# vrettasm/VGPA

Hardware: AMD Instinct MI355X
Metric: fwd+bwd sweeps/sec (free-energy+grad eval), Lorenz96 D=40 N=1000 (higher is better)
Workload: dtype f64; 1 GPU; Lorenz96 D=40, RK4, Np=1001 (BASELINE configs[2]); batch_per_gpu=512, kernels=mfma

## Files before the change

### vgpa_amd/csrc/energy.hip

```cpp
#include "vgpa_internal.h"
#include "energy_small.h"
#include "chol_wave.h"

namespace vgpa {
namespace {

constexpr int NT = 256;

__global__ void __launch_bounds__(NT) k_energy_1d(EnergyArgs a) {
  const int t = blockIdx.x * NT + threadIdx.x;
  const int prob = blockIdx.y;
  if (t >= a.Np) return;
  const size_t o = (size_t)prob * a.Np + t;
  const double la = a.A[(size_t)prob * a.strideA + t], ob = a.b[(size_t)prob * a.strideB + t], m = a.m[o], s = a.S[o];
  Energy1d r;
  const double th = a.theta_v ? a.theta_v[(size_t)prob * kMaxTheta] : a.theta[0];
  const double sg = a.sigma1_v ? a.sigma1_v[prob] : a.sigma1;
  if (a.model == VGPA_MODEL_OU) energy_1d<VGPA_MODEL_OU>(th, sg, la, ob, m, s, r);
  else energy_1d<VGPA_MODEL_DW>(th, sg, la, ob, m, s, r);
  if (a.hyp_only) { a.hyp[o] = r.hyp; return; }
  a.e_t[o] = r.e_t;
  a.Ef[o] = r.ef;
  if (a.Edf) a.Edf[o] = r.edf;
  a.dEm[o] = r.dm;
  a.dEs[o] = r.ds;
  if (a.hyp) a.hyp[o] = r.hyp;
}

__global__ void __launch_bounds__(64) k_energy_l63(EnergyArgs a) {
  const int t = blockIdx.x * 64 + threadIdx.x;
  const int prob = blockIdx.y;
  if (t >= a.Np) return;
  const size_t o = (size_t)prob * a.Np + t;
  const double* At = a.A + (size_t)prob * a.strideA + (size_t)t * 9;
  const double* bt = a.b + (size_t)prob * a.strideB + (size_t)t * 3;
  const double* mt = a.m + o * 3;
  const double* St = a.S + o * 9;
  double Av[9], bv[3], mv[3], Sv[9], isg[3];
  const double* th = a.theta_v ? a.theta_v + (size_t)prob * kMaxTheta : a.theta;
  const double* isgp = a.isg + (size_t)prob * a.isg_stride;
#pragma unroll
  for (int e = 0; e < 9; e++) { Av[e] = At[e]; Sv[e] = St[e]; }
#pragma unroll
  for (int i = 0; i < 3; i++) { bv[i] = bt[i]; mv[i] = mt[i]; isg[i] = isgp[i]; }
  EnergyL63 r;
  if (a.hyp) energy_l63<true>(th, isg, Av, bv, mv, Sv, r); else energy_l63<false>(th, isg, Av, bv, mv, Sv, r);
  if (a.hyp_only) {
    double* hp = a.hyp + o * 6;
#pragma unroll
    for (int i = 0; i < 6; i++) hp[i] = r.hyp[i];
    return;
  }
  a.e_t[o] = r.e_t;
  double* dm = a.dEm + o * 3;
  dm[0] = r.dm[0]; dm[1] = r.dm[1]; dm[2] = r.dm[2];
  double* ds = a.dEs + o * 9;
  ds[0] = r.ds[0]; ds[1] = r.ds[1]; ds[2] = r.ds[2];
  ds[3] = r.ds[1]; ds[4] = r.ds[3]; ds[5] = r.ds[4];
  ds[6] = r.ds[2]; ds[7] = r.ds[4]; ds[8] = r.ds[5];
  double* ef = a.Ef + o * 3;
  ef[0] = r.ef[0]; ef[1] = r.ef[1]; ef[2] = r.ef[2];
  if (a.hyp) {
    double* hp = a.hyp + o * 6;
#pragma unroll
    for (int i = 0; i < 6; i++) hp[i] = r.hyp[i];
  }
  if (a.Edf) {
    double* e = a.Edf + o * 9;
    const double vS = th[0], vR = th[1], vB = th[2];
    e[0] = -vS; e[1] = vS; e[2] = 0.0;
    e[3] = vR - mv[2]; e[4] = -1.0; e[5] = -mv[0];
    e[6] = mv[1]; e[7] = mv[0]; e[8] = -vB;
  }
}

__device__ __forceinline__ int wrap(int i, int n) { return i < 0 ? i + n : (i >= n ? i - n : i); }

__device__ __forceinline__ void wave_sync() {
  __builtin_amdgcn_fence(__ATOMIC_RELEASE, "wavefront");
  __builtin_amdgcn_wave_barrier();
  __builtin_amdgcn_fence(__ATOMIC_ACQUIRE, "wavefront");
}

__device__ __forceinline__ double lane_value(double v, int j) {
  const int lo = __builtin_amdgcn_readlane(__double2loint(v), j);
  const int hi = __builtin_amdgcn_readlane(__double2hiint(v), j);
  return __hiloint2double(hi, lo);
}

using cholw::chol_panel_pivots;
using cholw::rsqrt_pos;

__device__ __forceinline__ double wave_sum(double v) {
#pragma unroll
  for (int o = 32; o > 0; o >>= 1) v += __shfl_xor(v, o, 64);
  return v;
}

template <int NB>
struct WaveGemmGeo {
  static constexpr int NQ = NB / 4, REM = NB % 4, G = REM ? 4 / REM : 0;
  static constexpr int NLEFT = REM ? (NB + G - 1) / G : 0;
  static constexpr int NU = NB * NQ + NLEFT;
};

template <int NB, int MODE, int TRI = 0>
__device__ __forceinline__ void wave_gemm(const double* __restrict__ Aop, const double* __restrict__ Bm, int LD,
                                          double (&acc)[WaveGemmGeo<NB>::NU], const double* __restrict__ bscale = nullptr) {
  using g = WaveGemmGeo<NB>;
  const int l = threadIdx.x & 63, r4 = l >> 4, c4 = l & 3, b = (l >> 2) & 3;
  constexpr int rem = g::REM ? g::REM : 1;
#pragma unroll
  for (int u = 0; u < g::NU; u++) acc[u] = 0.0;
  const double* pa = Aop + r4 * LD + c4;
  const double* pb = Bm + r4 * LD;
  const int colq = l & 15;
  const int coll = 4 * (4 * g::NQ + b % rem) + c4;
  const int ileft = b / rem;
#pragma unroll
  for (int kk = 0; kk < NB; kk++) {
    const double bs = bscale ? bscale[4 * kk + r4] : 1.0;
    double bq[g::NQ > 0 ? g::NQ : 1];
#pragma unroll
    for (int q = 0; q < g::NQ; q++)
      if (kk >= 4 * q) bq[q] = bscale ? bs * pb[kk * 4 * LD + 16 * q + colq] : pb[kk * 4 * LD + 16 * q + colq];
    double bl = 0.0;
    if (g::NLEFT > 0 && kk >= 4 * g::NQ) bl = bscale ? bs * pb[kk * 4 * LD + coll] : pb[kk * 4 * LD + coll];
#pragma unroll
    for (int I = 0; I < NB; I++) {
      if (MODE == 1 && kk < I) continue;
      bool any = false;
#pragma unroll
      for (int q = 0; q < g::NQ; q++) any = any || (kk >= 4 * q && !(TRI == 1 && 4 * q + 3 < I) && !(TRI == 2 && 4 * q > I));
      if (!any) continue;
      const double af = pa[kk * 4 * LD + 4 * I];
#pragma unroll
      for (int q = 0; q < g::NQ; q++)
        if (kk >= 4 * q && !(TRI == 1 && 4 * q + 3 < I) && !(TRI == 2 && 4 * q > I)) acc[q * NB + I] = __builtin_amdgcn_mfma_f64_4x4x4f64(af, bq[q], acc[q * NB + I], 0, 0, 0);
    }
    if (g::NLEFT > 0 && kk >= 4 * g::NQ) {
#pragma unroll
      for (int v = 0; v < g::NLEFT; v++) {
        if (MODE == 1 && kk < v * g::G) continue;
        if (TRI == 2 && v * g::G + g::G - 1 < 4 * g::NQ) continue;
        int ib = v * g::G + ileft;
        ib = ib < NB ? ib : NB - 1;
        const double af = pa[kk * 4 * LD + 4 * ib];
        acc[NB * g::NQ + v] = __builtin_amdgcn_mfma_f64_4x4x4f64(af, bl, acc[NB * g::NQ + v], 0, 0, 0);
      }
    }
  }
}

template <int NB>
__device__ __forceinline__ void wave_gemm_elem(int u, int& row, int& col, bool& ok) {
  using g = WaveGemmGeo<NB>;
  const int l = threadIdx.x & 63, r4 = l >> 4, c4 = l & 3, b = (l >> 2) & 3;
  constexpr int rem = g::REM ? g::REM : 1;
  int Ib, Jb;
  if (u < NB * g::NQ) {
    const int q = u / NB;
    Ib = u - q * NB; Jb = 4 * q + b; ok = true;
  } else {
    const int v = u - NB * g::NQ;
    Ib = v * g::G + b / rem; Jb = 4 * g::NQ + b % rem;
    ok = (b < g::G * g::REM) && (Ib < NB);
  }
  row = 4 * Ib + r4; col = 4 * Jb + c4;
}

struct L96Lds {
  double *Lm, *Gm, *mv, *bv, *am, *sg, *vv, *dl, *qq, *rd;
};

__host__ __device__ inline int l96_dp(int D) { return 4 * ((D + 3) / 4); }
__host__ __device__ inline int l96_ld(int D) { return l96_dp(D) + 1; }
__host__ __device__ inline size_t l96_lds_doubles(int D) {
  return (size_t)2 * l96_dp(D) * l96_ld(D) + 7 * (size_t)l96_dp(D) + (2 * D + 1) + 8 + 4 * (size_t)l96_dp(D);
}

template <int NB>
__global__ void __launch_bounds__(64) k_energy_l96(EnergyArgs a) {
  extern __shared__ __attribute__((aligned(16))) double smem[];
  const int D = a.D, M = 2 * D + 1;
  constexpr int Dp = 4 * NB, LD = Dp + 1;
  const int l = threadIdx.x;
  const long long wid = blockIdx.x;
  const int prob = (int)(wid / a.Np), t = (int)(wid - (long long)prob * a.Np);
  const size_t o = (size_t)prob * a.Np + t;
  L96Lds S;
  S.Lm = smem; S.Gm = S.Lm + Dp * LD; S.mv = S.Gm + Dp * LD; S.bv = S.mv + Dp; S.am = S.bv + Dp; S.sg = S.am + Dp;
  S.dl = S.sg + Dp; S.qq = S.dl + Dp; S.rd = S.qq + Dp; S.vv = S.rd + Dp;
  const double* At = a.A + (size_t)prob * a.strideA + (size_t)t * D * D;
  const double* St = a.S + o * D * D;
  const double theta = a.theta_v ? lds_const(a.theta_v, prob * kMaxTheta) : a.theta[0];
  const double kappa = 1.05 * D, c = D + kappa;
  const bool act = l < D;
  const bool pad = l < Dp;
  const int li = pad ? l : Dp - 1;

  for (int e = l; e < Dp * LD; e += 64) { S.Lm[e] = 0.0; S.Gm[e] = 0.0; }
  if (pad) { S.mv[l] = 0.0; S.bv[l] = 0.0; S.sg[l] = 0.0; S.am[l] = 0.0; S.dl[l] = 0.0; S.qq[l] = 0.0; S.rd[l] = 1.0; }
  wave_sync();
  {
    constexpr int EPL = (Dp * Dp + 63) / 64;
    const int DD = D * D;
    const unsigned magic = ((1u << 20) + (unsigned)D - 1u) / (unsigned)D;
#pragma unroll
    for (int q0 = 0; q0 < EPL; q0 += 9) {
      double sv[9], av[9];
#pragma unroll
      for (int u = 0; u < 9; u++) {
        const int e = l + 64 * (q0 + u);
        const bool in = (q0 + u < EPL) && (e < DD);
        sv[u] = in ? St[e] : 0.0;
        av[u] = in ? At[e] : 0.0;
      }
#pragma unroll
      for (int u = 0; u < 9; u++) {
        const int e = l + 64 * (q0 + u);
        if ((q0 + u < EPL) && (e < DD)) {
          const int r = (int)(((unsigned)e * magic) >> 20), cc = e - r * D;
          S.Lm[r * LD + cc] = c * sv[u];
          S.Gm[cc * LD + r] = av[u];
        }
      }
    }
  }
  if (l >= D && pad) S.Lm[l * LD + l] = 1.0;
  if (act) { S.mv[l] = a.m[o * D + l]; S.bv[l] = a.b[(size_t)prob * a.strideB + (size_t)t * D + l]; S.sg[l] = a.isg[(size_t)prob * a.isg_stride + l]; }
  wave_sync();

  const int r4 = l >> 4, c4 = l & 3, b = (l >> 2) & 3;
  bool bad = false;
  double myrd = 1.0;
  const double* lrow_b = S.Lm + (4 * b + c4) * LD + r4;
  double* lout_b = S.Lm + (4 * b + r4) * LD + c4;
#pragma unroll
  for (int p = 0; p < NB; p++) {
    const int j0 = 4 * p;
    if (p > 0) {
      const double* brow = S.Lm + (j0 + c4) * LD + r4;
#pragma unroll
      for (int u = 0; p + 4 * u < NB; u++) {
        const bool full = p + 4 * u + 3 < NB;
        const bool rowok = full || (p + 4 * u + b < NB);
        const double* arow = full ? lrow_b + 4 * (p + 4 * u) * LD
                                  : S.Lm + (4 * (rowok ? p + 4 * u + b : NB - 1) + c4) * LD + r4;
        double uacc = 0.0;
#pragma unroll
        for (int kk = 0; kk < p; kk++) uacc = __builtin_amdgcn_mfma_f64_4x4x4f64(arow[4 * kk], brow[4 * kk], uacc, 0, 0, 0);
        if (rowok) lout_b[4 * (p + 4 * u) * LD + j0] -= uacc;
      }
      wave_sync();
    }
    chol_panel_pivots<LD>(S.Lm, myrd, j0, l, li, pad);
    wave_sync();
  }
  if (pad) S.rd[l] = myrd;
  wave_sync();
  bad = __any(!(myrd > 0.0 && myrd < __builtin_inf()));
  if (bad) {
    if (l == 0) atomicOr(a.status + prob, 1);
    return;
  }

  double* xdiag = S.vv + (2 * D + 1) + 7;
  if (l < NB) {
    const double* tb = S.Lm + (4 * l) * LD + 4 * l;
    const double x00 = S.rd[4 * l], x11 = S.rd[4 * l + 1], x22 = S.rd[4 * l + 2], x33 = S.rd[4 * l + 3];
    const double t10 = tb[LD], t20 = tb[2 * LD], t21 = tb[2 * LD + 1], t30 = tb[3 * LD], t31 = tb[3 * LD + 1], t32 = tb[3 * LD + 2];
    const double x10 = -(t10 * x00) * x11;
    const double x21 = -(t21 * x11) * x22;
    const double x32 = -(t32 * x22) * x33;
    const double x20 = -(t20 * x00 + t21 * x10) * x22;
    const double x31 = -(t31 * x11 + t32 * x21) * x33;
    const double x30 = -(t30 * x00 + t31 * x10 + t32 * x20) * x33;
    double* xo = xdiag + 16 * l;
    xo[0] = x00; xo[1] = 0.0; xo[2] = 0.0; xo[3] = 0.0;
    xo[4] = x10; xo[5] = x11; xo[6] = 0.0; xo[7] = 0.0;
    xo[8] = x20; xo[9] = x21; xo[10] = x22; xo[11] = 0.0;
    xo[12] = x30; xo[13] = x31; xo[14] = x32; xo[15] = x33;
  }
  {
    double s = 0.0;
#pragma unroll
    for (int k = 0; k < Dp; k++) s = __builtin_fma(S.Gm[k * LD + li], S.mv[k], s);
    if (act) { S.am[l] = s; if (a.Am) a.Am[o * D + l] = s; }
    double acc[WaveGemmGeo<NB>::NU];
    wave_gemm<NB, 0>(S.Gm, S.Lm, LD, acc);
    wave_sync();
#pragma unroll
    for (int u = 0; u < WaveGemmGeo<NB>::NU; u++) {
      int row, col; bool ok;
      wave_gemm_elem<NB>(u, row, col, ok);
      if (ok) S.Gm[row * LD + col] = acc[u];
    }
  }
  wave_sync();

  double vplus = 0.0, vminus = 0.0, v0 = 0.0, r0sq = 0.0;
  const bool hyper = a.hyp != nullptr;
  {
    auto col_of = [&](int q) { return q == 0 ? 0 : (q <= D ? q - 1 : q - 1 - D); };
    auto sgn_of = [&](int q) { return q == 0 ? 0.0 : (q <= D ? 1.0 : -1.0); };
    auto chi = [&](int q, int i) { return S.mv[i] + sgn_of(q) * S.Lm[i * LD + col_of(q)]; };
    const int jc = act ? l : 0;
    const int pP = 1 + jc, pM = 1 + D + jc;
    const int pPm = pP - 1, pPp = pP + 1;
    const int pMm = pM - 1, pMp = wrap(pM + 1, M);
    double am2 = chi(pPm, D - 2), am1 = chi(pPm, D - 1), a0 = chi(pP, 0), a1 = chi(pP, 1);
    double bm2 = chi(pMm, D - 2), bm1 = chi(pMm, D - 1), b0 = chi(pM, 0), b1 = chi(pM, 1);
    const double* lcol = S.Lm + jc;
    const double* gcol = S.Gm + jc;
#pragma unroll
    for (int i = 0; i < Dp; i++) {
      if (i >= D) break;
      const double gi = gcol[i * LD], ami = S.am[i], bvi = S.bv[i], sgi = S.sg[i];
      const double ra = ((a1 - am2) * am1 - a0 + theta) + (ami + gi) - bvi;
      const double rb = ((b1 - bm2) * bm1 - b0 + theta) + (ami - gi) - bvi;
      vplus = __builtin_fma(sgi, ra * ra, vplus);
      vminus = __builtin_fma(sgi, rb * rb, vminus);
      if (hyper && act) S.Gm[i * LD + jc] = ra * ra + rb * rb;
      am2 = am1; am1 = a0; a0 = a1;
      bm2 = bm1; bm1 = b0; b0 = b1;
      const int in = i + 2;
      if (in < D) {
        const double mi = S.mv[in], li2 = lcol[in * LD];
        a1 = mi + li2; b1 = mi - li2;
      } else {
        a1 = chi(pPp, in - D); b1 = chi(pMp, in - D);
      }
    }
    if (act) {
      const int i = l;
      const double xm2 = (i >= 2) ? S.mv[i - 2] : chi(M - 1, D - 2 + i);
      const double xm1 = (i >= 1) ? S.mv[i - 1] : chi(M - 1, D - 1);
      const double x1 = (i + 1 < D) ? S.mv[i + 1] : chi(1, 0);
      const double r0 = ((x1 - xm2) * xm1 - S.mv[i] + theta) + S.am[i] - S.bv[i];
      r0sq = r0 * r0;
      v0 = S.sg[i] * r0sq;
    }
    v0 = wave_sum(v0);
  }
  const double w0 = kappa / c, w1 = 1.0 / (2.0 * c);
  if (hyper) {
    wave_sync();
    if (act) {
      double sm = 0.0;
      for (int j = 0; j < D; j++) sm += S.Gm[l * LD + j];
      const int i = l, ip1 = wrap(i + 1, D), im1 = wrap(i - 1, D), im2 = wrap(i - 2, D);
      const double efi = (St[ip1 * D + im1] - St[im2 * D + im1]) + (S.mv[ip1] - S.mv[im2]) * S.mv[im1] - S.mv[i] + theta;
      double* hp = a.hyp + o * 2 * D;
      hp[i] = efi + S.am[i] - S.bv[i];
      hp[D + i] = w0 * r0sq + w1 * sm;
    }
  }
  const double e_part = act ? (vplus + vminus) : 0.0;
  const double e_t = 0.5 * (w0 * v0 + w1 * wave_sum(e_part));
  if (act) {
    S.dl[l] = w1 * (vplus - vminus);
    S.qq[l] = 0.5 * c * (w1 * (vplus + vminus)) - e_t;
  }
  if (l == 0) a.e_t[o] = e_t;
  wave_sync();

  const double* l4_a = S.Lm + c4 * LD + r4;
  const double* xd_a = xdiag + 4 * c4 + r4;
  const double* xd_d = xdiag + 4 * r4 + c4;
#pragma unroll
  for (int I = 0; I < NB; I++) {
    const double* arow = l4_a + 4 * I * LD;
    const double xd = xd_a[16 * I];
    const double xdd = xd_d[16 * I];
#pragma unroll
    for (int u = 0; 4 * u < NB; u++) {
      const int Jb = 4 * u + b;
      const bool colok = (4 * u + 3 < NB) || (Jb < NB);
      double* xcol = S.Gm + r4 * LD + 4 * (colok ? Jb : NB - 1) + c4;
      double xo = 0.0;
      if (4 * u <= I) {
        double tacc = 0.0;
#pragma unroll
        for (int K = 4 * u; K < I; K++) tacc = __builtin_amdgcn_mfma_f64_4x4x4f64(arow[4 * K], xcol[4 * K * LD], tacc, 0, 0, 0);
        const double prod = __builtin_amdgcn_mfma_f64_4x4x4f64(xd, tacc, 0.0, 0, 0, 0);
        xo = (Jb < I) ? -prod : ((Jb == I) ? xdd : 0.0);
      }
      if (colok) xcol[4 * I * LD] = xo;
    }
    wave_sync();
  }

  {
    double s = 0.0;
    for (int k = 0; k < Dp; k++) s = __builtin_fma(S.Gm[k * LD + li], S.dl[k], s);
    if (act) a.dEm[o * D + l] = 0.5 * c * s;
  }
  double* ds = a.dEs + o * D * D;
  {
    double acc[WaveGemmGeo<NB>::NU];
    wave_gemm<NB, 1>(S.Gm, S.Gm, LD, acc, S.qq);
#pragma unroll
    for (int u = 0; u < WaveGemmGeo<NB>::NU; u++) {
      int row, col; bool ok;
      wave_gemm_elem<NB>(u, row, col, ok);
      if (ok && row < D && col < D && (row <= col || !a.ds_upper)) ds[row * D + col] = 0.5 * c * acc[u];
    }
  }

  if (act) {
    const int i = l, ip1 = wrap(i + 1, D), im1 = wrap(i - 1, D), im2 = wrap(i - 2, D);
    const double cxx = St[ip1 * D + im1] - St[im2 * D + im1];
    a.Ef[o * D + i] = cxx + (S.mv[ip1] - S.mv[im2]) * S.mv[im1] - S.mv[i] + theta;
  }
  if (a.Edf) {
    double* ed = a.Edf + o * D * D;
    for (int e = l; e < D * D; e += 64) {
      const int k = e / D, j = e - k * D;
      const int kp1 = wrap(k + 1, D), km1 = wrap(k - 1, D), km2 = wrap(k - 2, D);
      double v = 0.0;
      if (j == k) v = -1.0;
      if (j == kp1) v = S.mv[km1];
      if (j == km2) v = -S.mv[km1];
      if (j == km1) v = S.mv[kp1] - S.mv[km2];
      ed[e] = v;
    }
  }
}

__host__ __device__ inline bool l96r_compact(int D) { return (D + 3) / 4 == 10; }
__host__ __device__ inline size_t l96r_lds_doubles(int D) {
  const size_t dp = l96_dp(D);
  if (l96r_compact(D)) return dp * l96_ld(D) + 5 * dp;
  return dp * l96_ld(D) + 6 * dp + 9 * dp;
}
template <int R>
__device__ __forceinline__ double row_ror_blocks(double v) {
  typedef int i2_t __attribute__((ext_vector_type(2)));
  i2_t x = __builtin_bit_cast(i2_t, v), y;
  y[0] = __builtin_amdgcn_mov_dpp(x[0], 0x120 + 4 * R, 0xf, 0xf, false);
  y[1] = __builtin_amdgcn_mov_dpp(x[1], 0x120 + 4 * R, 0xf, 0xf, false);
  return __builtin_bit_cast(double, y);
}

struct TriRowTab { unsigned char r[2080]; };
constexpr TriRowTab make_tri_row_tab() {
  TriRowTab t{};
  int e = 0;
  for (int r = 0; r < 64; r++)
    for (int c = 0; c <= r; c++) t.r[e++] = (unsigned char)r;
  return t;
}
__device__ __constant__ TriRowTab kTriRow = make_tri_row_tab();

template <int NB, bool TG = false>
__global__ void __launch_bounds__(64) __attribute__((amdgpu_waves_per_eu(NB <= 10 ? 3 : 2, NB <= 10 ? 3 : 2))) k_energy_l96_r(EnergyArgs a) {
  extern __shared__ __attribute__((aligned(16))) double smem[];
  const int D = a.D, M = 2 * D + 1;
  constexpr int Dp = 4 * NB, LD = Dp + 1, NUU = (NB + 3) / 4;
  const int l = threadIdx.x;
  const long long wid = blockIdx.x;
  const int prob = (int)(wid / a.Np);
  const int t = (int)(wid - (long long)prob * a.Np);
  const size_t o = (size_t)prob * a.Np + t;
  L96Lds S;
  constexpr bool CMP = (NB == 10);
  S.Lm = smem; S.Gm = nullptr; S.mv = S.Lm + Dp * LD; S.bv = S.mv + Dp; S.am = S.bv + Dp; S.sg = nullptr;
  S.dl = S.am + Dp; S.qq = S.dl + Dp; S.rd = CMP ? nullptr : S.qq + Dp; S.vv = CMP ? nullptr : S.rd + Dp;
  double* pv = S.vv;
  double* pw = CMP ? nullptr : pv + 4 * Dp;
  double* gb2 = CMP ? nullptr : pw + 4 * Dp;
  double* xdiag = pv;
  auto cg2 = [&](int j) -> double* { return S.Lm + j * LD + Dp; };
  auto cps = [&](int minus, int j) -> double* { return S.Lm + (4 + 2 * minus + (j >= 20 ? 1 : 0)) * LD + (j >= 20 ? j : 20 + j); };
  auto cxd = [&](int I, int r, int c) -> double* { return S.Lm + ((I < 6 ? 0 : 4) + r) * LD + 4 * (I < 6 ? I + 4 : I - 1) + c; };
  const double* At = a.A + (size_t)prob * a.strideA + (size_t)t * D * D;
  const bool spk = a.s_packed != 0;
  const int PK = tri_off(D);
  const double* St = a.S + o * (spk ? PK : D * D);
  const double theta = a.theta_v ? lds_const(a.theta_v, prob * kMaxTheta) : a.theta[0];
  const double kappa = 1.05 * D, c = D + kappa;
  const bool act = l < D;
  const bool pad = l < Dp;
  const int li = pad ? l : Dp - 1;
  const int r4 = l >> 4, c4 = l & 3, b = (l >> 2) & 3;

  constexpr int NUE = 0;
  double af[NUU][NB];
  const int klim = (D - r4 + 3) >> 2;
  auto load_af = [&](int u) {
    const int row = 16 * u + (l & 15);
    const double* ap = At + row * D + r4;
    const int kl = row < D ? klim : 0;
#pragma unroll
    for (int K = 0; K < NB; K++) af[u][K] = (K < kl) ? ap[4 * K] : 0.0;
  };

  double sxa = 0.0, sxb = 0.0, v_m = 0.0, v_b = 0.0, v_sg = 0.0;
  double nsxa = 0.0, nsxb = 0.0;
  const int f_ip1 = wrap(l + 1, D), f_im1 = wrap(l - 1, D), f_im2 = wrap(l - 2, D);
  if (act) v_sg = a.isg[(size_t)prob * a.isg_stride + l];
  auto load_vectors = [&]() {
    if (act) {
      sxa = St[f_ip1 * D + f_im1];
      sxb = St[f_im2 * D + f_im1];
      v_m = a.m[o * D + l];
      v_b = a.b[(size_t)prob * a.strideB + (size_t)t * D + l];
    }
  };
  constexpr int EPK = (Dp * (Dp + 1) / 2 + 63) / 64;
  double sv[EPK];
  int rr[EPK];
  auto request = [&](int tn) {
    const size_t on = (size_t)prob * a.Np + tn;
    const double* Sn = a.S + on * PK;
#pragma unroll
    for (int q = 0; q < EPK; q++) {
      const int e = l + 64 * q;
      sv[q] = e < PK ? Sn[e] : 0.0;
      rr[q] = kTriRow.r[e < PK ? e : 0];
    }
    if (act) {
      nsxa = Sn[tri_idx(f_ip1, f_im1)];
      nsxb = Sn[tri_idx(f_im2, f_im1)];
      v_m = a.m[on * D + l];
      v_b = a.b[(size_t)prob * a.strideB + (size_t)tn * D + l];
    }
  };
  if (spk) request(t);

  if (spk) {
    if (D != Dp) {
      for (int e = l; e < Dp * LD; e += 64) S.Lm[e] = 0.0;
      wave_sync();
    }
    sxa = nsxa; sxb = nsxb;
#pragma unroll
    for (int q = 0; q < EPK; q++) {
      const int e = l + 64 * q;
      if (e < PK) {
        const int r = rr[q];
        S.Lm[r * LD + (e - tri_off(r))] = c * sv[q];
      }
    }
  } else if (D == Dp) {
    constexpr int RCH = Dp <= 44 ? Dp : 32;
    const double* sp = St + li;
#pragma unroll
    for (int q0 = 0; q0 < Dp; q0 += RCH) {
      double sv[RCH];
#pragma unroll
      for (int u = 0; u < RCH; u++) sv[u] = (q0 + u < Dp) ? sp[(q0 + u) * Dp] : 0.0;
      if (q0 == 0) load_vectors();
      if (pad) {
#pragma unroll
        for (int u = 0; u < RCH; u++)
          if (q0 + u < Dp) S.Lm[(q0 + u) * LD + l] = c * sv[u];
      }
    }
  } else {
    load_vectors();
    for (int e = l; e < Dp * LD; e += 64) S.Lm[e] = 0.0;
    wave_sync();
    constexpr int EPL = (Dp * Dp + 63) / 64;
    constexpr int CH = (NB <= 11) ? EPL : 13;
    const int DD = D * D;
    const unsigned magic = ((1u << 20) + (unsigned)D - 1u) / (unsigned)D;
#pragma unroll
    for (int q0 = 0; q0 < EPL; q0 += CH) {
      double sv[CH];
#pragma unroll
      for (int u = 0; u < CH; u++) {
        const int e = l + 64 * (q0 + u);
        const bool in = (q0 + u < EPL) && (e < DD);
        sv[u] = in ? St[e] : 0.0;
      }
#pragma unroll
      for (int u = 0; u < CH; u++) {
        const int e = l + 64 * (q0 + u);
        if ((q0 + u < EPL) && (e < DD)) {
          const int r = (int)(((unsigned)e * magic) >> 20), cc = e - r * D;
          S.Lm[r * LD + cc] = c * sv[u];
        }
      }
    }
  }
  if (l >= D && pad) S.Lm[l * LD + l] = 1.0;
  if (pad) { S.mv[l] = v_m; S.bv[l] = v_b; S.am[l] = 0.0; }
  wave_sync();

  bool bad = false;
  double myrd = 1.0;
  const double* lrow_b = S.Lm + (4 * b + c4) * LD + r4;
  double* lout_b = S.Lm + (4 * b + r4) * LD + c4;
#pragma unroll
  for (int p = 0; p < NB; p++) {
    const int j0 = 4 * p;
    if (p > 0) {
      const double* brow = S.Lm + (j0 + c4) * LD + r4;
#pragma unroll
      for (int u = 0; p + 4 * u < NB; u++) {
        const bool full = p + 4 * u + 3 < NB;
        const bool rowok = full || (p + 4 * u + b < NB);
        const double* arow = full ? lrow_b + 4 * (p + 4 * u) * LD
                                  : S.Lm + (4 * (rowok ? p + 4 * u + b : NB - 1) + c4) * LD + r4;
        double uacc = 0.0;
#pragma unroll
        for (int kk = 0; kk < p; kk++) uacc = __builtin_amdgcn_mfma_f64_4x4x4f64(arow[4 * kk], brow[4 * kk], uacc, 0, 0, 0);
        if (rowok) lout_b[4 * (p + 4 * u) * LD + j0] -= uacc;
      }
      wave_sync();
    }
    chol_panel_pivots<LD>(S.Lm, myrd, j0, l, li, pad);
    wave_sync();
  }
  if (!CMP && pad) S.rd[l] = myrd;
  wave_sync();
  bad = __any(!(myrd > 0.0 && myrd < __builtin_inf()));
  if (bad) {
    if (l == 0) atomicOr(a.status + prob, 1);
    return;
  }
#pragma unroll
  for (int u = NUE; u < NUU; u++) load_af(u);

  double amr[NUU], gacc[NUU][NB];
#pragma unroll
  for (int u = 0; u < NUU; u++) {
    amr[u] = 0.0;
#pragma unroll
    for (int J = 0; J < NB; J++) gacc[u][J] = 0.0;
  }
#pragma unroll
  for (int pass = 0; pass < (NUE < NUU ? 2 : 1); pass++) {
    const int u0 = pass == 0 ? 0 : NUE, u1 = pass == 0 ? NUE : NUU;
#pragma unroll
    for (int K = 0; K < NB; K++) {
      const double mk = S.mv[4 * K + r4];
#pragma unroll
      for (int u = u0; u < u1; u++) amr[u] = __builtin_amdgcn_mfma_f64_4x4x4f64(af[u][K], mk, amr[u], 0, 0, 0);
      const double* lk = S.Lm + (4 * K + r4) * LD + c4;
#pragma unroll
      for (int J = 0; J <= K; J++) {
        const double lf = lk[4 * J];
#pragma unroll
        for (int u = u0; u < u1; u++) gacc[u][J] = __builtin_amdgcn_mfma_f64_4x4x4f64(af[u][K], lf, gacc[u][J], 0, 0, 0);
      }
    }
  }
#pragma unroll
  for (int u = 0; u < NUU; u++) {
    const int i = 16 * u + 4 * b + r4;
    if (c4 == 0 && i < D) { S.am[i] = amr[u]; if (!TG && a.Am) a.Am[o * D + i] = amr[u]; }
  }
  if constexpr (TG) wave_sync();

  if constexpr (!TG) {
#pragma unroll
  for (int u = 0; u < NUU; u++) {
    if (u == 0 || (16 * u <= Dp - 1 && 16 * u + 15 >= Dp - 4)) {
      const int i = 16 * u + 4 * b + r4;
      if constexpr (CMP) {
        if (i == D - 1) {
#pragma unroll
          for (int J = 0; J < NB; J++) *cg2(4 * J + c4) = gacc[u][J];
        }
      }
      double* gdst = (i == 0) ? S.dl : ((i == 1) ? S.qq : ((i == D - 1 && !CMP) ? gb2 : nullptr));
      if (gdst) {
#pragma unroll
        for (int J = 0; J < NB; J++) gdst[4 * J + c4] = gacc[u][J];
      }
    }
  }
  }
  double tg_edge = 0.0;
  if constexpr (TG) {
    const double w0 = kappa / c, w1 = 1.0 / (2.0 * c);
    auto col_of = [&](int q) { return q == 0 ? 0 : (q <= D ? q - 1 : q - 1 - D); };
    auto sgn_of = [&](int q) { return q == 0 ? 0.0 : (q <= D ? 1.0 : -1.0); };
    auto chi = [&](int q, int i) { return S.mv[i] + sgn_of(q) * S.Lm[i * LD + col_of(q)]; };
    const int jc = act ? l : 0;
    const int pP = 1 + jc, pM = 1 + D + jc;
    const int pPm = pP - 1, pPp = pP + 1;
    const int pMm = pM - 1, pMp = wrap(pM + 1, M);
    const double P0 = chi(pPm, D - 2), P1 = chi(pPm, D - 1), P2 = chi(pP, 0), P3 = chi(pP, 1), P4 = chi(pP, 2);
    const double N0 = chi(pMm, D - 2), N1 = chi(pMm, D - 1), N2 = chi(pM, 0), N3 = chi(pM, 1), N4 = chi(pM, 2);
    const double Q0 = chi(pP, D - 3), Q1 = chi(pP, D - 2), Q2 = chi(pP, D - 1), Q3 = chi(pPp, 0);
    const double R0 = chi(pM, D - 3), R1 = chi(pM, D - 2), R2 = chi(pM, D - 1), R3 = chi(pMp, 0);
    double bsum = 0.0;
    {
      const double lin = S.am[0] - S.bv[0];
      bsum += lane_value(v_sg, 0) * ((((P3 - P0) * P1 - P2 + theta) + lin) + (((N3 - N0) * N1 - N2 + theta) + lin));
    }
    {
      const double lin = S.am[1] - S.bv[1];
      bsum += lane_value(v_sg, 1) * ((((P4 - P1) * P2 - P3 + theta) + lin) + (((N4 - N1) * N2 - N3 + theta) + lin));
    }
    {
      const double lin = S.am[D - 1] - S.bv[D - 1];
      bsum += lane_value(v_sg, D - 1) * ((((Q3 - Q0) * Q1 - Q2 + theta) + lin) + (((R3 - R0) * R1 - R2 + theta) + lin));
    }
    double part = 0.0;
    if (act) {
      const int i = l;
      const double xm2 = (i >= 2) ? S.mv[i - 2] : chi(M - 1, D - 2 + i);
      const double xm1 = (i >= 1) ? S.mv[i - 1] : chi(M - 1, D - 1);
      const double x1 = (i + 1 < D) ? S.mv[i + 1] : chi(1, 0);
      const double r0 = ((x1 - xm2) * xm1 - S.mv[i] + theta) + S.am[i] - S.bv[i];
      part += w1 * bsum + w0 * (v_sg * r0);
    }
    tg_edge = part;
  }
  double vp[NB], vm[NB];
  double tgi = 0.0;
#pragma unroll
  for (int J = 0; J < NB; J++) { vp[J] = 0.0; vm[J] = 0.0; }
  {
#pragma clang fp contract(fast)
#pragma unroll
  for (int u = 0; u < NUU; u++) {
    const int i = 16 * u + 4 * b + r4;
    const bool ok = (i >= 2) && (i <= D - 2);
    const int ir = ok ? i : 2;
    const double mm2 = S.mv[ir - 2], mm1 = S.mv[ir - 1], m0 = S.mv[ir], m1 = S.mv[ir + 1];
    const double sgr = __shfl(v_sg, ir, 64);
    const double bvi = S.bv[ir], sgi = ok ? sgr : 0.0, ami = amr[u];
    const double dm = m1 - mm2;
    const double base = dm * mm1 - m0 + theta + ami - bvi;
    const double* lp = S.Lm + (ir - 2) * LD + c4;
#pragma unroll
    for (int J = 0; J < NB; J++) {
      const double e2 = lp[4 * J], e1 = lp[LD + 4 * J], e0 = lp[2 * LD + 4 * J], ep = lp[3 * LD + 4 * J];
      const double gi = gacc[u][J];
      const double dl = ep - e2;
      const double ev = base + dl * e1;
      const double od = dm * e1 + (dl * mm1 + (gi - e0));
      vp[J] = vp[J] + sgi * (ev * ev + od * od);
      vm[J] = vm[J] + sgi * (ev * od);
      if constexpr (TG) tgi = tgi + ((4 * J + c4 < D) ? sgi : 0.0) * ev;
      if (J == NB / 2 - 1 || J == NB - 1) __builtin_amdgcn_sched_barrier(0);
    }
  }
  }
  if constexpr (TG) {
    const double part = wave_sum(tg_edge + 2.0 * (1.0 / (2.0 * c)) * tgi);
    if (l == 0) a.tg[o] = part;
    return;
  }
  {
    double rp[NB], rm[NB];
#pragma unroll
    for (int J = 0; J < NB; J++) {
      rp[J] = __builtin_amdgcn_mfma_f64_4x4x4f64(1.0, vp[J], 0.0, 0, 0, 0);
      rm[J] = __builtin_amdgcn_mfma_f64_4x4x4f64(1.0, vm[J], 0.0, 0, 0, 0);
    }
    if constexpr (CMP) {
#pragma unroll
      for (int J = 0; J < NB; J++) {
        const double p1 = rp[J] + row_ror_blocks<1>(rp[J]), m1 = rm[J] + row_ror_blocks<1>(rm[J]);
        rp[J] = p1 + row_ror_blocks<2>(p1);
        rm[J] = m1 + row_ror_blocks<2>(m1);
      }
      wave_sync();
      if (r4 == 0 && b == 0) {
#pragma unroll
        for (int J = 0; J < NB; J++) {
          *cps(0, 4 * J + c4) = rp[J];
          *cps(1, 4 * J + c4) = rm[J];
        }
      }
    } else
    if (r4 == 0) {
#pragma unroll
      for (int J = 0; J < NB; J++) {
        pv[b * Dp + 4 * J + c4] = rp[J];
        pw[b * Dp + 4 * J + c4] = rm[J];
      }
    }
  }
  wave_sync();

  double vplus = 0.0, vminus = 0.0, v0 = 0.0;
  {
    auto col_of = [&](int q) { return q == 0 ? 0 : (q <= D ? q - 1 : q - 1 - D); };
    auto sgn_of = [&](int q) { return q == 0 ? 0.0 : (q <= D ? 1.0 : -1.0); };
    auto chi = [&](int q, int i) { return S.mv[i] + sgn_of(q) * S.Lm[i * LD + col_of(q)]; };
    const int jc = act ? l : 0;
    {
      double s1, s2;
      if constexpr (CMP) { s1 = *cps(0, jc); s2 = *cps(1, jc); }
      else {
        s1 = (pv[jc] + pv[Dp + jc]) + (pv[2 * Dp + jc] + pv[3 * Dp + jc]);
        s2 = (pw[jc] + pw[Dp + jc]) + (pw[2 * Dp + jc] + pw[3 * Dp + jc]);
      }
      vplus = s1 + 2.0 * s2;
      vminus = s1 - 2.0 * s2;
    }
    const int pP = 1 + jc, pM = 1 + D + jc;
    const int pPm = pP - 1, pPp = pP + 1;
    const int pMm = pM - 1, pMp = wrap(pM + 1, M);
    {
      const double P0 = chi(pPm, D - 2), P1 = chi(pPm, D - 1), P2 = chi(pP, 0), P3 = chi(pP, 1), P4 = chi(pP, 2);
      const double N0 = chi(pMm, D - 2), N1 = chi(pMm, D - 1), N2 = chi(pM, 0), N3 = chi(pM, 1), N4 = chi(pM, 2);
      const double Q0 = chi(pP, D - 3), Q1 = chi(pP, D - 2), Q2 = chi(pP, D - 1), Q3 = chi(pPp, 0);
      const double R0 = chi(pM, D - 3), R1 = chi(pM, D - 2), R2 = chi(pM, D - 1), R3 = chi(pMp, 0);
      const double g0 = S.dl[jc], g1 = S.qq[jc], g2 = CMP ? *cg2(jc) : gb2[jc];
      {
        const double ami = S.am[0], bvi = S.bv[0], sgi = lane_value(v_sg, 0);
        const double ra = ((P3 - P0) * P1 - P2 + theta) + (ami + g0) - bvi;
        const double rb = ((N3 - N0) * N1 - N2 + theta) + (ami - g0) - bvi;
        vplus = __builtin_fma(sgi, ra * ra, vplus);
        vminus = __builtin_fma(sgi, rb * rb, vminus);
      }
      {
        const double ami = S.am[1], bvi = S.bv[1], sgi = lane_value(v_sg, 1);
        const double ra = ((P4 - P1) * P2 - P3 + theta) + (ami + g1) - bvi;
        const double rb = ((N4 - N1) * N2 - N3 + theta) + (ami - g1) - bvi;
        vplus = __builtin_fma(sgi, ra * ra, vplus);
        vminus = __builtin_fma(sgi, rb * rb, vminus);
      }
      {
        const double ami = S.am[D - 1], bvi = S.bv[D - 1], sgi = lane_value(v_sg, D - 1);
        const double ra = ((Q3 - Q0) * Q1 - Q2 + theta) + (ami + g2) - bvi;
        const double rb = ((R3 - R0) * R1 - R2 + theta) + (ami - g2) - bvi;
        vplus = __builtin_fma(sgi, ra * ra, vplus);
        vminus = __builtin_fma(sgi, rb * rb, vminus);
      }
    }
    if (act) {
      const int i = l;
      const double xm2 = (i >= 2) ? S.mv[i - 2] : chi(M - 1, D - 2 + i);
      const double xm1 = (i >= 1) ? S.mv[i - 1] : chi(M - 1, D - 1);
      const double x1 = (i + 1 < D) ? S.mv[i + 1] : chi(1, 0);
      const double r0 = ((x1 - xm2) * xm1 - S.mv[i] + theta) + S.am[i] - S.bv[i];
      v0 = v_sg * (r0 * r0);
    }
    v0 = wave_sum(v0);
  }
  const double w0 = kappa / c, w1 = 1.0 / (2.0 * c);
  const double e_part = act ? (vplus + vminus) : 0.0;
  const double e_t = 0.5 * (w0 * v0 + w1 * wave_sum(e_part));
  wave_sync();
  if (pad) {
    S.dl[l] = act ? w1 * (vplus - vminus) : 0.0;
    S.qq[l] = act ? 0.5 * c * (w1 * (vplus + vminus)) - e_t : 0.0;
  }
  if (l == 0) a.e_t[o] = e_t;
  const int l4 = l < NB ? 4 * l : 0;
  const double rd0 = CMP ? __shfl(myrd, l4, 64) : 0.0, rd1 = CMP ? __shfl(myrd, l4 + 1, 64) : 0.0;
  const double rd2 = CMP ? __shfl(myrd, l4 + 2, 64) : 0.0, rd3 = CMP ? __shfl(myrd, l4 + 3, 64) : 0.0;
  if (l < NB) {
    const double* tb = S.Lm + (4 * l) * LD + 4 * l;
    const double x00 = CMP ? rd0 : S.rd[4 * l], x11 = CMP ? rd1 : S.rd[4 * l + 1], x22 = CMP ? rd2 : S.rd[4 * l + 2], x33 = CMP ? rd3 : S.rd[4 * l + 3];
    const double t10 = tb[LD], t20 = tb[2 * LD], t21 = tb[2 * LD + 1], t30 = tb[3 * LD], t31 = tb[3 * LD + 1], t32 = tb[3 * LD + 2];
    const double x10 = -(t10 * x00) * x11;
    const double x21 = -(t21 * x11) * x22;
    const double x32 = -(t32 * x22) * x33;
    const double x20 = -(t20 * x00 + t21 * x10) * x22;
    const double x31 = -(t31 * x11 + t32 * x21) * x33;
    const double x30 = -(t30 * x00 + t31 * x10 + t32 * x20) * x33;
    if constexpr (CMP) {
      double* x0 = cxd(l, 0, 0);
      x0[0] = x00; x0[1] = 0.0; x0[2] = 0.0; x0[3] = 0.0;
      x0[LD] = x10; x0[LD + 1] = x11; x0[LD + 2] = 0.0; x0[LD + 3] = 0.0;
      x0[2 * LD] = x20; x0[2 * LD + 1] = x21; x0[2 * LD + 2] = x22; x0[2 * LD + 3] = 0.0;
      x0[3 * LD] = x30; x0[3 * LD + 1] = x31; x0[3 * LD + 2] = x32; x0[3 * LD + 3] = x33;
    } else {
    double* xo = xdiag + 16 * l;
    xo[0] = x00; xo[1] = 0.0; xo[2] = 0.0; xo[3] = 0.0;
    xo[4] = x10; xo[5] = x11; xo[6] = 0.0; xo[7] = 0.0;
    xo[8] = x20; xo[9] = x21; xo[10] = x22; xo[11] = 0.0;
    xo[12] = x30; xo[13] = x31; xo[14] = x32; xo[15] = x33;
    }
  }
  wave_sync();

  const double* l4_a = S.Lm + c4 * LD + r4;
  const double* xd_a = xdiag + 4 * c4 + r4;
  const double* xd_d = xdiag + 4 * r4 + c4;
#pragma unroll
  for (int I = 0; I < NB; I++) {
    const double* arow = l4_a + 4 * I * LD;
    const double xd = CMP ? *cxd(I, c4, r4) : xd_a[16 * I];
    const double xdd = CMP ? *cxd(I, r4, c4) : xd_d[16 * I];
    double xo[NUU];
#pragma unroll
    for (int u = 0; u < NUU; u++) {
      const int Jb = 4 * u + b;
      const bool colok = (4 * u + 3 < NB) || (Jb < NB);
      const double* xcol = S.Lm + r4 * LD + 4 * (colok ? Jb : NB - 1) + c4;
      xo[u] = 0.0;
      if (4 * u <= I) {
        double tacc = 0.0;
#pragma unroll
        for (int K = 4 * u; K < I; K++) tacc = __builtin_amdgcn_mfma_f64_4x4x4f64(arow[4 * K], xcol[4 * K * LD], tacc, 0, 0, 0);
        const double prod = __builtin_amdgcn_mfma_f64_4x4x4f64(xd, tacc, 0.0, 0, 0, 0);
        xo[u] = (Jb < I) ? -prod : ((Jb == I) ? xdd : 0.0);
      }
    }
#pragma unroll
    for (int u = 0; u < NUU; u++) {
      const int Jb = 4 * u + b;
      const bool colok = (4 * u + 3 < NB) || (Jb < NB);
      if (colok && (!CMP || Jb <= I)) S.Lm[(4 * I + r4) * LD + 4 * Jb + c4] = xo[u];
    }
    wave_sync();
  }

  {
    double s = 0.0;
    if constexpr (CMP) {
      const bool z0 = li < 4, z1 = li < 8;
#pragma unroll
      for (int k = 0; k < 8; k++) s = __builtin_fma((k < 4 ? z0 : z1) ? S.Lm[k * LD + li] : 0.0, S.dl[k], s);
      for (int k = 8; k < Dp; k++) s = __builtin_fma(S.Lm[k * LD + li], S.dl[k], s);
    } else
    for (int k = 0; k < Dp; k++) s = __builtin_fma(S.Lm[k * LD + li], S.dl[k], s);
    if (act) a.dEm[o * D + l] = 0.5 * c * s;
  }
  double* ds = a.dEs + o * D * D;
  {
    double acc[WaveGemmGeo<NB>::NU];
    if (a.ds_packed) {
      using gg = WaveGemmGeo<NB>;
      double* dsp = a.dEs + o * PK;
      wave_gemm<NB, 1, 2>(S.Lm, S.Lm, LD, acc, S.qq);
#pragma unroll
      for (int u = 0; u < gg::NU; u++) {
        if (u < NB * gg::NQ && 4 * (u / NB) > u % NB) continue;
        if (u >= NB * gg::NQ && (u - NB * gg::NQ) * gg::G + gg::G - 1 < 4 * gg::NQ) continue;
        int row, col; bool ok;
        wave_gemm_elem<NB>(u, row, col, ok);
        if (ok && row < D && col <= row) dsp[tri_off(row) + col] = 0.5 * c * acc[u];
      }
    } else if (a.ds_upper) {
      wave_gemm<NB, 1, 1>(S.Lm, S.Lm, LD, acc, S.qq);
#pragma unroll
      for (int u = 0; u < WaveGemmGeo<NB>::NU; u++) {
        if (u < NB * WaveGemmGeo<NB>::NQ && 4 * (u / NB) + 3 < u % NB) continue;
        int row, col; bool ok;
        wave_gemm_elem<NB>(u, row, col, ok);
        if (ok && row < D && col < D && row <= col) ds[row * D + col] = 0.5 * c * acc[u];
      }
    } else {
      wave_gemm<NB, 1>(S.Lm, S.Lm, LD, acc, S.qq);
#pragma unroll
      for (int u = 0; u < WaveGemmGeo<NB>::NU; u++) {
        int row, col; bool ok;
        wave_gemm_elem<NB>(u, row, col, ok);
        if (ok && row < D && col < D) ds[row * D + col] = 0.5 * c * acc[u];
      }
    }
  }

  if (act) {
    const int i = l, ip1 = wrap(i + 1, D), im1 = wrap(i - 1, D), im2 = wrap(i - 2, D);
    const double cxx = sxa - sxb;
    a.Ef[o * D + i] = cxx + (S.mv[ip1] - S.mv[im2]) * S.mv[im1] - S.mv[i] + theta;
  }
  if (a.Edf) {
    double* ed = a.Edf + o * D * D;
    for (int e = l; e < D * D; e += 64) {
      const int k = e / D, j = e - k * D;
      const int kp1 = wrap(k + 1, D), km1 = wrap(k - 1, D), km2 = wrap(k - 2, D);
      double v = 0.0;
      if (j == k) v = -1.0;
      if (j == kp1) v = S.mv[km1];
      if (j == km2) v = -S.mv[km1];
      if (j == km1) v = S.mv[kp1] - S.mv[km2];
      ed[e] = v;
    }
  }
}

__global__ void __launch_bounds__(NT) k_edf_dense(EnergyArgs a) {
  const int D = a.D;
  const int t = blockIdx.x, prob = blockIdx.y;
  const size_t o = (size_t)prob * a.Np + t;
  const double* mv = a.m + o * D;
  double* ed = a.Edf + o * D * D;
  const double* th = a.theta_v ? a.theta_v + (size_t)prob * kMaxTheta : a.theta;
  for (int e = threadIdx.x; e < D * D; e += NT) {
    const int k = e / D, j = e - k * D;
    double v = 0.0;
    if (a.model == VGPA_MODEL_L96) {
      const int kp1 = wrap(k + 1, D), km1 = wrap(k - 1, D), km2 = wrap(k - 2, D);
      if (j == k) v = -1.0;
      if (j == kp1) v = mv[km1];
      if (j == km2) v = -mv[km1];
      if (j == km1) v = mv[kp1] - mv[km2];
    } else if (a.model == VGPA_MODEL_L63) {
      const double vS = th[0], vR = th[1], vB = th[2];
      const double tab[9] = {-vS, vS, 0.0, vR - mv[2], -1.0, -mv[0], mv[1], mv[0], -vB};
      v = tab[e];
    } else if (a.model == VGPA_MODEL_OU) {
      v = -th[0];
    } else {
      v = 4.0 * (th[0] - 3.0 * (mv[0] * mv[0] + a.S[o]));
    }
    ed[e] = v;
  }
}

}
}

namespace vgpa {

hipError_t launch_energy(const EnergyArgs& a, hipStream_t st) {
  if (a.model == VGPA_MODEL_OU || a.model == VGPA_MODEL_DW) {
    dim3 grid((a.Np + NT - 1) / NT, a.batch);
    hipLaunchKernelGGL(k_energy_1d, grid, dim3(NT), 0, st, a);
  } else if (a.model == VGPA_MODEL_L63) {
    dim3 grid((a.Np + 63) / 64, a.batch);
    hipLaunchKernelGGL(k_energy_l63, grid, dim3(64), 0, st, a);
  } else if (a.model == VGPA_MODEL_L96) {
    if (a.D < 4 || a.D > kMaxSmallD) return hipErrorInvalidValue;
    const bool one_matrix = (a.hyp == nullptr);
    if (a.tg && !one_matrix) return hipErrorInvalidValue;
    size_t lds = (one_matrix ? l96r_lds_doubles(a.D) : l96_lds_doubles(a.D)) * sizeof(double);
    const long long nwaves = (long long)a.Np * a.batch;
    if (nwaves > 0x7fffffffLL) return hipErrorInvalidValue;
#define VGPA_L96_CASE(NBV)                                                                                          \
  case NBV:                                                                                                         \
    if (lds > 48 * 1024)                                                                                            \
      (void)hipFuncSetAttribute(one_matrix ? (const void*)k_energy_l96_r<NBV> : (const void*)k_energy_l96<NBV>,       \
                                hipFuncAttributeMaxDynamicSharedMemorySize, (int)lds);                                \
    if (a.tg) {                                                                                                     \
      if (lds > 48 * 1024)                                                                                          \
        (void)hipFuncSetAttribute((const void*)k_energy_l96_r<NBV, true>, hipFuncAttributeMaxDynamicSharedMemorySize, (int)lds); \
      hipLaunchKernelGGL((k_energy_l96_r<NBV, true>), dim3((unsigned)nwaves), dim3(64), lds, st, a);                  \
    } else                                                                                                          \
    if (one_matrix) hipLaunchKernelGGL(k_energy_l96_r<NBV>, dim3((unsigned)nwaves), dim3(64), lds, st, a);          \
    else hipLaunchKernelGGL(k_energy_l96<NBV>, dim3((unsigned)nwaves), dim3(64), lds, st, a);                        \
    break;
    switch ((a.D + 3) / 4) {
      VGPA_L96_CASE(1) VGPA_L96_CASE(2) VGPA_L96_CASE(3) VGPA_L96_CASE(4) VGPA_L96_CASE(5) VGPA_L96_CASE(6)
      VGPA_L96_CASE(7) VGPA_L96_CASE(8) VGPA_L96_CASE(9) VGPA_L96_CASE(10) VGPA_L96_CASE(11) VGPA_L96_CASE(12)
      VGPA_L96_CASE(13) VGPA_L96_CASE(14) VGPA_L96_CASE(15) VGPA_L96_CASE(16)
      default: return hipErrorInvalidValue;
    }
#undef VGPA_L96_CASE
  } else {
    return hipErrorInvalidValue;
  }
  return hipGetLastError();
}

hipError_t launch_edf(const EnergyArgs& a, hipStream_t st) {
  dim3 grid(a.Np, a.batch);
  hipLaunchKernelGGL(k_edf_dense, grid, dim3(NT), 0, st, a);
  return hipGetLastError();
}

}
```

Measured before the change: 23030 sweeps/s.

## Fuse dE/dm matvec into dEs MFMA gemm and force LDS operand loads

The separate per-lane scalar FMA loop that computed dE/dm as a column dot product with S.dl is replaced. The same product is now accumulated with extra MFMA ops inside the wave_gemm that already streams those L columns for dEs, which removes a second pass over the shared matrix. It also hoists B/A operand fragments into registers in the Cholesky update and inverse loops. Where a compile-time check finds the access pattern free of bank conflicts, it loads those operands through volatile address-space-3 pointers, presumably to get ds_read_b64 codegen. The volatile loads may stop the compiler from reordering or merging them, and the extra MFMAs lengthen the gemm's dependency chain.

After: 23260 sweeps/s, median of 6. About the same (+1.0%).

```diff
diff --git a/vgpa_amd/csrc/energy.hip b/vgpa_amd/csrc/energy.hip
--- a/vgpa_amd/csrc/energy.hip
+++ b/vgpa_amd/csrc/energy.hip
@@ -97,6 +97,22 @@
   return v;
 }
 
+typedef const volatile double __attribute__((address_space(3)))* frag_ptr;
+template <bool V> struct OpndPtr { typedef const double* type; };
+template <> struct OpndPtr<true> { typedef frag_ptr type; };
+constexpr bool b64_conflict_free(int LD, bool rowk) {
+  for (int h = 0; h < 2; h++) {
+    int e[8] = {0, 0, 0, 0, 0, 0, 0, 0};
+    int n = 0;
+    for (int r = 2 * h; r < 2 * h + 2; r++)
+      for (int c = 0; c < 4; c++) e[n++] = rowk ? c * LD + r : r * LD + c;
+    for (int i = 0; i < 8; i++)
+      for (int j = i + 1; j < 8; j++)
+        if ((e[i] - e[j]) % 32 == 0) return false;
+  }
+  return true;
+}
+
 template <int NB>
 struct WaveGemmGeo {
   static constexpr int NQ = NB / 4, REM = NB % 4, G = REM ? 4 / REM : 0;
@@ -104,15 +120,21 @@
   static constexpr int NU = NB * NQ + NLEFT;
 };
 
-template <int NB, int MODE, int TRI = 0>
+template <int NB, int MODE, int TRI = 0, bool B64A = false>
 __device__ __forceinline__ void wave_gemm(const double* __restrict__ Aop, const double* __restrict__ Bm, int LD,
-                                          double (&acc)[WaveGemmGeo<NB>::NU], const double* __restrict__ bscale = nullptr) {
+                                          double (&acc)[WaveGemmGeo<NB>::NU], const double* __restrict__ bscale = nullptr,
+                                          const double* __restrict__ dvec = nullptr, double* __restrict__ dm = nullptr) {
   using g = WaveGemmGeo<NB>;
   const int l = threadIdx.x & 63, r4 = l >> 4, c4 = l & 3, b = (l >> 2) & 3;
   constexpr int rem = g::REM ? g::REM : 1;
 #pragma unroll
   for (int u = 0; u < g::NU; u++) acc[u] = 0.0;
+  if (dvec) {
+#pragma unroll
+    for (int q = 0; q <= g::NQ; q++) dm[q] = 0.0;
+  }
   const double* pa = Aop + r4 * LD + c4;
+  const typename OpndPtr<B64A>::type pf = (typename OpndPtr<B64A>::type)pa;
   const double* pb = Bm + r4 * LD;
   const int colq = l & 15;
   const int coll = 4 * (4 * g::NQ + b % rem) + c4;
@@ -120,12 +142,21 @@
 #pragma unroll
   for (int kk = 0; kk < NB; kk++) {
     const double bs = bscale ? bscale[4 * kk + r4] : 1.0;
+    const double dk = dvec ? dvec[4 * kk + r4] : 0.0;
     double bq[g::NQ > 0 ? g::NQ : 1];
 #pragma unroll
     for (int q = 0; q < g::NQ; q++)
-      if (kk >= 4 * q) bq[q] = bscale ? bs * pb[kk * 4 * LD + 16 * q + colq] : pb[kk * 4 * LD + 16 * q + colq];
+      if (kk >= 4 * q) {
+        const double raw = pb[kk * 4 * LD + 16 * q + colq];
+        bq[q] = bscale ? bs * raw : raw;
+        if (dvec) dm[q] = __builtin_amdgcn_mfma_f64_4x4x4f64(raw, dk, dm[q], 0, 0, 0);
+      }
     double bl = 0.0;
-    if (g::NLEFT > 0 && kk >= 4 * g::NQ) bl = bscale ? bs * pb[kk * 4 * LD + coll] : pb[kk * 4 * LD + coll];
+    if (g::NLEFT > 0 && kk >= 4 * g::NQ) {
+      const double raw = pb[kk * 4 * LD + coll];
+      bl = bscale ? bs * raw : raw;
+      if (dvec) dm[g::NQ] = __builtin_amdgcn_mfma_f64_4x4x4f64(raw, dk, dm[g::NQ], 0, 0, 0);
+    }
 #pragma unroll
     for (int I = 0; I < NB; I++) {
       if (MODE == 1 && kk < I) continue;
@@ -133,7 +164,7 @@
 #pragma unroll
       for (int q = 0; q < g::NQ; q++) any = any || (kk >= 4 * q && !(TRI == 1 && 4 * q + 3 < I) && !(TRI == 2 && 4 * q > I));
       if (!any) continue;
-      const double af = pa[kk * 4 * LD + 4 * I];
+      const double af = pf[kk * 4 * LD + 4 * I];
 #pragma unroll
       for (int q = 0; q < g::NQ; q++)
         if (kk >= 4 * q && !(TRI == 1 && 4 * q + 3 < I) && !(TRI == 2 && 4 * q > I)) acc[q * NB + I] = __builtin_amdgcn_mfma_f64_4x4x4f64(af, bq[q], acc[q * NB + I], 0, 0, 0);
@@ -597,7 +628,10 @@
   for (int p = 0; p < NB; p++) {
     const int j0 = 4 * p;
     if (p > 0) {
-      const double* brow = S.Lm + (j0 + c4) * LD + r4;
+      const typename OpndPtr<b64_conflict_free(LD, true)>::type brow = (typename OpndPtr<b64_conflict_free(LD, true)>::type)(S.Lm + (j0 + c4) * LD + r4);
+      double bk[NB];
+#pragma unroll
+      for (int kk = 0; kk < p; kk++) bk[kk] = brow[4 * kk];
 #pragma unroll
       for (int u = 0; p + 4 * u < NB; u++) {
         const bool full = p + 4 * u + 3 < NB;
@@ -606,7 +640,7 @@
                                   : S.Lm + (4 * (rowok ? p + 4 * u + b : NB - 1) + c4) * LD + r4;
         double uacc = 0.0;
 #pragma unroll
-        for (int kk = 0; kk < p; kk++) uacc = __builtin_amdgcn_mfma_f64_4x4x4f64(arow[4 * kk], brow[4 * kk], uacc, 0, 0, 0);
+        for (int kk = 0; kk < p; kk++) uacc = __builtin_amdgcn_mfma_f64_4x4x4f64(arow[4 * kk], bk[kk], uacc, 0, 0, 0);
         if (rowok) lout_b[4 * (p + 4 * u) * LD + j0] -= uacc;
       }
       wave_sync();
@@ -634,12 +668,13 @@
 #pragma unroll
   for (int pass = 0; pass < (NUE < NUU ? 2 : 1); pass++) {
     const int u0 = pass == 0 ? 0 : NUE, u1 = pass == 0 ? NUE : NUU;
+    if (u0 == u1) continue;
 #pragma unroll
     for (int K = 0; K < NB; K++) {
       const double mk = S.mv[4 * K + r4];
 #pragma unroll
       for (int u = u0; u < u1; u++) amr[u] = __builtin_amdgcn_mfma_f64_4x4x4f64(af[u][K], mk, amr[u], 0, 0, 0);
-      const double* lk = S.Lm + (4 * K + r4) * LD + c4;
+      const typename OpndPtr<b64_conflict_free(LD, false)>::type lk = (typename OpndPtr<b64_conflict_free(LD, false)>::type)(S.Lm + (4 * K + r4) * LD + c4);
 #pragma unroll
       for (int J = 0; J <= K; J++) {
         const double lf = lk[4 * J];
@@ -881,7 +916,10 @@
   const double* xd_d = xdiag + 4 * r4 + c4;
 #pragma unroll
   for (int I = 0; I < NB; I++) {
-    const double* arow = l4_a + 4 * I * LD;
+    const typename OpndPtr<b64_conflict_free(LD, true)>::type arow = (typename OpndPtr<b64_conflict_free(LD, true)>::type)(l4_a + 4 * I * LD);
+    double ak[NB];
+#pragma unroll
+    for (int K = 0; K < I; K++) ak[K] = arow[4 * K];
     const double xd = CMP ? *cxd(I, c4, r4) : xd_a[16 * I];
     const double xdd = CMP ? *cxd(I, r4, c4) : xd_d[16 * I];
     double xo[NUU];
@@ -894,7 +932,7 @@
       if (4 * u <= I) {
         double tacc = 0.0;
 #pragma unroll
-        for (int K = 4 * u; K < I; K++) tacc = __builtin_amdgcn_mfma_f64_4x4x4f64(arow[4 * K], xcol[4 * K * LD], tacc, 0, 0, 0);
+        for (int K = 4 * u; K < I; K++) tacc = __builtin_amdgcn_mfma_f64_4x4x4f64(ak[K], xcol[4 * K * LD], tacc, 0, 0, 0);
         const double prod = __builtin_amdgcn_mfma_f64_4x4x4f64(xd, tacc, 0.0, 0, 0, 0);
         xo[u] = (Jb < I) ? -prod : ((Jb == I) ? xdd : 0.0);
       }
@@ -908,24 +946,30 @@
     wave_sync();
   }
 
-  {
-    double s = 0.0;
-    if constexpr (CMP) {
-      const bool z0 = li < 4, z1 = li < 8;
-#pragma unroll
-      for (int k = 0; k < 8; k++) s = __builtin_fma((k < 4 ? z0 : z1) ? S.Lm[k * LD + li] : 0.0, S.dl[k], s);
-      for (int k = 8; k < Dp; k++) s = __builtin_fma(S.Lm[k * LD + li], S.dl[k], s);
-    } else
-    for (int k = 0; k < Dp; k++) s = __builtin_fma(S.Lm[k * LD + li], S.dl[k], s);
-    if (act) a.dEm[o * D + l] = 0.5 * c * s;
-  }
+  double dmu[WaveGemmGeo<NB>::NQ + 1];
+  auto store_dm = [&]() {
+    using gg = WaveGemmGeo<NB>;
+    constexpr int rem = gg::REM ? gg::REM : 1;
+    if (c4 == 0) {
+#pragma unroll
+      for (int q = 0; q < gg::NQ; q++) {
+        const int i = 16 * q + 4 * b + r4;
+        if (i < D) a.dEm[o * D + i] = 0.5 * c * dmu[q];
+      }
+      if (gg::NLEFT > 0) {
+        const int i = 4 * (4 * gg::NQ + b) + r4;
+        if (b < rem && i < D) a.dEm[o * D + i] = 0.5 * c * dmu[gg::NQ];
+      }
+    }
+  };
   double* ds = a.dEs + o * D * D;
   {
     double acc[WaveGemmGeo<NB>::NU];
     if (a.ds_packed) {
       using gg = WaveGemmGeo<NB>;
       double* dsp = a.dEs + o * PK;
-      wave_gemm<NB, 1, 2>(S.Lm, S.Lm, LD, acc, S.qq);
+      wave_gemm<NB, 1, 2, b64_conflict_free(LD, false)>(S.Lm, S.Lm, LD, acc, S.qq, S.dl, dmu);
+      store_dm();
 #pragma unroll
       for (int u = 0; u < gg::NU; u++) {
         if (u < NB * gg::NQ && 4 * (u / NB) > u % NB) continue;
@@ -935,7 +979,8 @@
         if (ok && row < D && col <= row) dsp[tri_off(row) + col] = 0.5 * c * acc[u];
       }
     } else if (a.ds_upper) {
-      wave_gemm<NB, 1, 1>(S.Lm, S.Lm, LD, acc, S.qq);
+      wave_gemm<NB, 1, 1, b64_conflict_free(LD, false)>(S.Lm, S.Lm, LD, acc, S.qq, S.dl, dmu);
+      store_dm();
 #pragma unroll
       for (int u = 0; u < WaveGemmGeo<NB>::NU; u++) {
         if (u < NB * WaveGemmGeo<NB>::NQ && 4 * (u / NB) + 3 < u % NB) continue;
@@ -944,7 +989,8 @@
         if (ok && row < D && col < D && row <= col) ds[row * D + col] = 0.5 * c * acc[u];
       }
     } else {
-      wave_gemm<NB, 1>(S.Lm, S.Lm, LD, acc, S.qq);
+      wave_gemm<NB, 1, 0, b64_conflict_free(LD, false)>(S.Lm, S.Lm, LD, acc, S.qq, S.dl, dmu);
+      store_dm();
 #pragma unroll
       for (int u = 0; u < WaveGemmGeo<NB>::NU; u++) {
         int row, col; bool ok;
```
